# ut-amrl/nautilus

Measured on AMD Instinct MI355X. Metric: loop-closure candidate pairs/sec (1081-beam), higher is better.
Workload: dtype u16

## Files before the change

### nautilus_amd/csm.py

```python
import ctypes as C
import math

import numpy as np

from . import _lib
from ._lib import GridSpec, GridLayout, Search, Match, check, ptr

MATCH_DTYPE = np.dtype([("itheta", "<i4"), ("ix", "<i4"), ("iy", "<i4"), ("score", "<f4")])
assert MATCH_DTYPE.itemsize == C.sizeof(Match) == 16


def grid_spec(range_m=30.0, res=0.05, sigma=2.0, floor_p=1e-10, max_shift=40, cell_bits=16, skip_map=False, no_image=False):
    return GridSpec(float(range_m), float(res), float(sigma), float(floor_p), int(max_shift), int(cell_bits),
                    (_lib.NHIP_GRID_SKIP_MAP if skip_map else 0) | (_lib.NHIP_GRID_NO_IMAGE if no_image else 0), 0)


def search_spec(n_theta=61, nx=81, ny=81, theta_step=math.radians(1.0), exhaustive=False, dense=False, short_scans=False,
                exact_score=False, latency=False):
    flags = (_lib.NHIP_SEARCH_EXHAUSTIVE if exhaustive else 0) | (_lib.NHIP_SEARCH_DENSE if dense else 0) | \
            (_lib.NHIP_SEARCH_SHORT_SCANS if short_scans else 0) | (_lib.NHIP_SEARCH_EXACT_SCORE if exact_score else 0) | \
            (_lib.NHIP_SEARCH_LATENCY if latency else 0)
    return Search(int(n_theta), int(nx), int(ny), flags, float(theta_step))


# ... 174 lines not shown
    return np.asarray(matches)["itheta"] < 0


def gate_floor(spec, min_score, n_points):
    out = C.c_int32(0)
    check(_lib.load().nhip_csm_gate_floor(C.byref(spec), float(min_score), int(n_points), C.byref(out)))
    return out.value


def bnb_stats():
    a, b = C.c_uint64(0), C.c_uint64(0)
    check(_lib.load().nhip_bnb_stats(C.byref(a), C.byref(b)))
    return a.value, b.value


def bnb_stats_levels():
    v = (C.c_uint64 * 24)()
    check(_lib.load().nhip_bnb_stats_levels(v))
    return {"blocks_whole": v[0], "blocks_total": v[1], "candidates_refined": v[2], "sub_blocks": v[3],
            "clk_wave_phase3": v[4], "clk_origins": v[5], "clk_sub_bounds": v[6], "clk_exact": v[7],
            "clk_slowest_wave": v[8], "clk_seeds": v[9], "clk_bounds": v[10], "clk_wave_phase3_100MHz": v[11],
            "pairs_handed_over": v[12], "clk_wave_second_kernel": v[13], "pose_evals16": v[14],
            "pairs_settled_by_gate": v[15], "passes_l2_runs": v[16], "passes_per_cell_field": v[17],
            "passes_per_cell_capacity": v[18]}


def score_volume(scans, grids, src, slot, theta0, search, origin=(0, 0)):
    out = np.zeros((search.n_theta, search.nx, search.ny), dtype=np.int32)
    check(_lib.load().nhip_csm_scores(scans._h, grids._h, int(src), int(slot), float(theta0),
                                      int(origin[0]), int(origin[1]), C.byref(search), ptr(out)))
    return out


def match_to_transform(m, spec, search, theta0, origin=(0, 0)):
    tx = (origin[0] + int(m["ix"]) - (search.nx - 1) // 2) * spec.res
    ty = (origin[1] + int(m["iy"]) - (search.ny - 1) // 2) * spec.res
    th = theta0 + (int(m["itheta"]) - (search.n_theta - 1) // 2) * search.theta_step
    return np.float32(tx), np.float32(ty), np.float32(th)


class CorrelativeScanMatcher:

    def __init__(self, scanner_range, trans_range, low_res, high_res, sigma=2.0, cell_bits=16):
        self.params = _lib.CsmParams(float(scanner_range), float(trans_range), float(low_res), float(high_res),
                                     float(sigma), 1e-10, int(cell_bits), 0)

    def GetTransformation(self, pointcloud_a, pointcloud_b, rotation_a, rotation_b, rotation_restriction):
        a = np.ascontiguousarray(pointcloud_a, dtype=np.float32).reshape(-1, 2)
        b = np.ascontiguousarray(pointcloud_b, dtype=np.float32).reshape(-1, 2)
        score, tx, ty, th = C.c_double(0), C.c_float(0), C.c_float(0), C.c_float(0)
        check(_lib.load().nhip_csm_get_transformation(C.byref(self.params), ptr(a), len(a), ptr(b), len(b),
                                                      float(rotation_a), float(rotation_b), float(rotation_restriction),
                                                      C.byref(score), C.byref(tx), C.byref(ty), C.byref(th)))
        return score.value, ((np.float32(tx.value), np.float32(ty.value)), np.float32(th.value))


def last_launch():
    out = (C.c_int32 * 8)()
    check(_lib.load().nhip_csm_last_launch(out))
    form = {0: "fused", 1: "split, one round", 2: "split, rounds on one stream", 3: "split, rounds overlapped on the helper stream"}
    return {"form": form.get(out[0], "?"), "form_id": out[0], "pairs_per_round": out[1], "rounds_of_state": out[2],
            "rounds": out[3], "short_scans": bool(out[4]), "hand_over_kernel": bool(out[5]), "instrumented": bool(out[6] & 1),
            "l2_runs": bool(out[6] & 2), "n_pairs": out[7]}


def drop_in_cache_stats():
    v = [C.c_int64(0) for _ in range(4)]
    check(_lib.load().nhip_csm_cache_stats(*[C.byref(x) for x in v]))
    return dict(zip(("entries", "bytes", "hits", "misses"), (x.value for x in v)))


def drop_in_cache_clear():
    check(_lib.load().nhip_csm_cache_clear())


def drop_in_cache_configure(max_bytes):
    check(_lib.load().nhip_csm_cache_configure(int(max_bytes)))
```

### nautilus_amd/csrc/nhip_bnb.hip

```cpp
#include <atomic>
#include <mutex>
#include <type_traits>
#include <vector>

#ifndef NHIP_BNB_INSTR
#define NHIP_BNB_INSTR 0
#endif
#if NHIP_BNB_INSTR
#define csm_bnb_kernel csm_bnb_kernel_instr
#define csm_bnb_rot_kernel csm_bnb_rot_kernel_instr
#define launchers_product launchers_instr
#define BNB_STATS(P) ((P).stats)
#define BNB_TIMELINE(P) ((P).timeline)
#else
#define BNB_STATS(P) (static_cast<unsigned long long *>(nullptr))
#define BNB_TIMELINE(P) (static_cast<unsigned long long *>(nullptr))
#endif

#include "nhip_bnb_params.h"
#include "nhip_bnb_wave.h"
#include "nhip_bnb_origin.h"
#include "nhip_bnb_bounds.h"
#include "nhip_bnb_exact.h"

// ... 71 lines not shown
    return;
  }
#pragma unroll 1
  for (int q = 0; q < 4; q++) {
    const uint32_t b = q == 0 ? sb0 : (q == 1 ? sb1 : (q == 2 ? sb2 : sb3));
    if (b == 0u || b < best_sum_cached<GLOBAL>(best, bcopy)) continue;
    int dy, dx;
    const uint32_t total = sub_sums8(rsrc, pitch8, (uint32_t)P.hi_copy_bytes, org, nch, Y, X, q >> 1, q & 1, lane, &dy, &dx);
    const int32_t ix = BNB_B * X + BNB_B4 * (q & 1) + dx, iy = BNB_B * Y + BNB_B4 * (q >> 1) + dy;
    if (CB == 1) {
      const unsigned long long key = best_key(P, k, ix, iy, total, 8);
      wave_atomic_max(best, key, lane);
      if (GLOBAL) bcopy = max(bcopy, (uint32_t)(key >> 32));
    } else {
      n[3] += refine16<GLOBAL>(P, rsrc16, org, nch, n_pts, k, ix, iy, total, lane < 16, lane, best, bcopy);
    }
    n[2]++;
  }
}

struct PhaseClocks {
  long long org, strip, eval;
  uint32_t run_passes, cell_passes_field, cell_passes_full;
};

__device__ __forceinline__ void flush_stats(unsigned long long *stats, const uint32_t *n, int32_t pair, const PhaseClocks *clk) {
  if (n) {
    if (n[0]) atomicAdd(&stats[0], (unsigned long long)n[0]);
    if (n[1]) atomicAdd(&stats[2], (unsigned long long)n[1]);
    if (n[2]) atomicAdd(&stats[3], (unsigned long long)n[2]);
    if (n[3]) atomicAdd(&stats[14], (unsigned long long)n[3]);
    if (pair < BNB_STATS_PAIRS) atomicAdd(&stats[BNB_STATS_HEAD + pair], 4ull * n[0] + n[2]);
  }
  if (clk) {
    atomicAdd(&stats[5], (unsigned long long)clk->org);
    atomicAdd(&stats[6], (unsigned long long)clk->strip);
    atomicAdd(&stats[7], (unsigned long long)clk->eval);
    if (clk->run_passes) atomicAdd(&stats[16], (unsigned long long)clk->run_passes);
    if (clk->cell_passes_field) atomicAdd(&stats[17], (unsigned long long)clk->cell_passes_field);
    if (clk->cell_passes_full) atomicAdd(&stats[18], (unsigned long long)clk->cell_passes_full);
  }
}

template <int CB, bool GLOBAL, bool RUNS = false>
__device__ __forceinline__ void rotation_pass(const BnbParams &P, const PairCtx &C, int32_t k, uint32_t u0, uint32_t u1,
                                              unsigned long long m0, unsigned long long m1, int lane,
                                              unsigned long long *best, uint32_t *done, uint32_t *org,
                                              uint32_t (&n_work)[4], PhaseClocks &clk, uint32_t *runs = nullptr) {
  long long t_mark = 0;
  float cf, sf;
  rotation_k(P, C.pair, k, &cf, &sf);
  if (BNB_STATS(P)) t_mark = clock64();
  int32_t nrc = RUNS_NONE;
  const int32_t nch = cache_origins<RUNS>(P, C.pts, C.n_pts, cf, sf, C.cx, C.cy, lane, org, true, runs, RUNS && P.l2_runs != 0, &nrc);
  if (BNB_STATS(P)) clk.org += clock64() - t_mark;
  if (RUNS && BNB_STATS(P)) {
    clk.run_passes += nrc > 0 ? 1u : 0u;
    clk.cell_passes_field += nrc == RUNS_FIELD ? 1u : 0u;
    clk.cell_passes_full += nrc == RUNS_FULL ? 1u : 0u;
  }
  const __amdgpu_buffer_rsrc_t rsrc16 = CB == 1 ? uniform_rsrc(C.grid, P.grid_bytes + P.skip_bytes)
                                                : uniform_rsrc(C.grid + P.hi_offset + 2 * P.hi_copy_bytes, P.t16_bytes);
  const __amdgpu_buffer_rsrc_t rsrc = uniform_rsrc(C.grid + P.hi_offset, 2 * P.hi_copy_bytes);
  const uint32_t pitch8 = (uint32_t)P.hi_tpr;
  const __amdgpu_buffer_rsrc_t p4 = uniform_rsrc(C.grid + P.grid_bytes + P.skip_bytes + P.pool_bytes, P.pool4_bytes);
  while ((m0 | m1) != 0ull) {
    const int b0 = m0 ? (int)__builtin_ctzll(m0) : 64 + (int)__builtin_ctzll(m1);
    const int Y = b0 / NB, X0 = b0 - NB * Y;
    int len = 1;
    while (len < 3 && X0 + len < NB) {
      const int b = b0 + len;
      if (!(((b < 64 ? m0 >> b : m1 >> (b - 64)) & 1ull))) break;
      len++;
    }
    uint32_t sb[12];
    uint32_t bcopy = GLOBAL ? best_sum<true>(best) : 0u;
    if (P.levels >= 2) {
      if (BNB_STATS(P)) t_mark = clock64();
// ... 151 lines not shown
    }
    if ((uint32_t)(wbest >> 32) < (uint32_t)gfloor) wbest = 0ull;
  }
  uint32_t n_work[4] = {0u, 0u, 0u, 0u};
  PairCtx C;
  C.grid = grid;
  C.pts = pts;
  C.n_pts = n_pts;
  C.cx = cx;
  C.cy = cy;
  C.pair = pair;
  if (BY_ROT) {
    __syncthreads();
    uint32_t *org = s_org + wave * ORG_WAVE + lane;
    PhaseClocks clk = {0, 0, 0, 0u, 0u, 0u};
    long long t_busy = 0, t_wall = 0;
    const long long t_phase1 = BNB_STATS(P) ? clock64() : 0;
    if (BNB_TIMELINE(P) && threadIdx.x == 0 && pair < BNB_STATS_PAIRS) BNB_TIMELINE(P)[4 * pair + 1] = wall_clock64();
    const uint32_t xcd = bid & 7u;
    bool handed_over = false;
    enum { SEED, OWN };
    int state = SEED;
    bool heavy = false;
    for (;;) {
      bool have = false;
      int32_t k = 0;
      uint32_t u0 = 0u, u1 = 0u;
      unsigned long long m0 = 0ull, m1 = 0ull;
      uint32_t *done = nullptr;
      if (state == SEED) {
        if ((uint32_t)(wbest >> 32) != 0u) {
          const int32_t v = (int32_t)(wbest & 0xffu);
          const uint32_t ub = (uint32_t)(wbest >> 32);
          k = (int32_t)((uint32_t)wbest >> 8);
          u0 = v == lane ? ub : 0u;
          u1 = v == lane + 64 ? ub : 0u;
          m0 = v < 64 ? 1ull << v : 0ull;
          m1 = v < 64 ? 0ull : 1ull << (v - 64);
          done = s_U + k * 128;
          have = true;
        }
      } else if (state == OWN) {
        const int32_t rank = (int32_t)wave_fetch_add(s_qhead, 1u, lane);
        if (rank >= P.n_theta) break;
        k = (int32_t)s_order[rank];
        u0 = s_U[k * 128 + lane];
        u1 = s_U[k * 128 + 64 + lane];
        const uint32_t bsum = best_sum<false>(s_best);
        m0 = __ballot(u0 != 0u && u0 >= bsum);
        m1 = __ballot(u1 != 0u && u1 >= bsum && lane + 64 < NB * NB);
        if ((m0 | m1) == 0ull) continue;
        if (heavy && (uint32_t)rank >= P.keep_ranks) {
          const uint32_t lx = (xcd + (uint32_t)rank) & 7u;
          const uint32_t e = wave_fetch_add(P.rot_count + 8 * lx, 1u, lane);
          if (e < P.rot_cap) {
            if (lane < 4) {
              const unsigned long long M41 = (1ull << 41) - 1ull;
              const unsigned long long word = lane == 0   ? ((unsigned long long)(uint32_t)pair << 24) | (uint32_t)k
                                              : lane == 1 ? (m0 & M41)
                                              : lane == 2 ? ((m0 >> 41) | (m1 << 23)) & M41
                                                          : (m1 >> 18);
              P.rot_list[(size_t)lx * P.rot_cap + e].w[lane] = word;
            }
            handed_over = true;
            continue;
          }
        }
        have = true;
      }
      if (have) rotation_pass<CB, false>(P, C, k, u0, u1, m0, m1, lane, s_best, done, org, n_work, clk);
      if (state == SEED) {
        __syncthreads();
        if (BNB_TIMELINE(P) && threadIdx.x == 0 && pair < BNB_STATS_PAIRS) BNB_TIMELINE(P)[4 * pair + 2] = wall_clock64();
        if (BNB_STATS(P)) {
          t_busy = clock64();
          t_wall = wall_clock64();
        }
        for (int32_t kk = threadIdx.x; kk < P.n_theta; kk += THREADS) {
          const unsigned long long mine = s_kmax[kk];
          int32_t rank = 0;
          for (int32_t j = 0; j < P.n_theta; j++) rank += s_kmax[j] > mine ? 1 : 0;
          s_order[rank] = (uint32_t)kk;
        }
        if (P.rot_list || SPLIT) {
          const uint32_t bsum = best_sum<false>(s_best);
          uint32_t mine = 0u;
          for (int32_t kk = wave; kk < P.n_theta; kk += WAVES) {
            const uint32_t c0 = s_U[kk * 128 + lane], c1 = s_U[kk * 128 + 64 + lane];
            mine += (uint32_t)__builtin_popcountll(__ballot(c0 != 0u && c0 >= bsum)) +
                    (uint32_t)__builtin_popcountll(__ballot(c1 != 0u && c1 >= bsum && lane + 64 < NB * NB));
          }
          if (wave_leader(lane)) atomicAdd(s_qn, mine);
        }
        __syncthreads();
        if (SPLIT) {
          const uint32_t bsum = best_sum<false>(s_best);
          uint32_t *rows = P.ps_rows + (size_t)pair * (size_t)P.n_theta * 128u;
          uint32_t live = 0u;
          for (int32_t r = wave; r < P.n_theta; r += WAVES) {
            const uint32_t kk = s_order[r];
            const uint32_t kmax = (uint32_t)(s_kmax[kk] >> 32);
            if (kmax == 0u || kmax < bsum) break;
            live = (uint32_t)r + 1u;
            const uint32_t w1 = lane == 62 ? kmax : (lane == 63 ? kk : s_U[kk * 128 + 64 + lane]);
            rows[(size_t)r * 128u + lane] = s_U[kk * 128 + lane];
            rows[(size_t)r * 128u + 64 + lane] = w1;
          }
          if (live && wave_leader(lane)) atomicMax(s_qhead, live);
          __syncthreads();
          if (threadIdx.x == 0) {
            P.ps_count[pair] = *s_qn;
            P.ps_live[pair] = *s_qhead;
            P.ps_next[pair] = 0u;
          }
          break;
        }
        heavy = P.rot_list && *s_qn >= P.heavy_min;
        state = OWN;
      }
    }
    if (BNB_STATS(P) && lane == 0) {
      const long long now = clock64();
      atomicAdd(&BNB_STATS(P)[4], (unsigned long long)(now - t_busy));
      atomicAdd(&BNB_STATS(P)[11], (unsigned long long)(wall_clock64() - t_wall));
      flush_stats(BNB_STATS(P), nullptr, pair, &clk);
      atomicMax(s_slow, (unsigned long long)(now - t_busy));
      if (wave == 0) {
        atomicAdd(&BNB_STATS(P)[9], (unsigned long long)(t_busy - t_phase1));
        atomicAdd(&BNB_STATS(P)[10], (unsigned long long)(t_phase1 - t_start));
        if (handed_over) atomicAdd(&BNB_STATS(P)[12], 1ull);
      }
    }
  } else {
  if ((uint32_t)(wbest >> 32) != 0u) {
      const int32_t k = (int32_t)((uint32_t)wbest >> 8), v = (int32_t)(wbest & 0xffu);
      const int Y = v / NB, X = v - NB * Y;
// ... 169 lines not shown
constexpr int ORDER_THREADS = 256;
__global__ __launch_bounds__(ORDER_THREADS) void csm_bnb_order_spread_kernel(BnbParams P) {
  const int32_t p = (int32_t)(blockIdx.x * ORDER_THREADS + threadIdx.x);
  if (p >= P.n_pairs) return;
  const int32_t extra_slots = P.ps_work_stride - P.pairs_per_xcd;
  const int32_t home = p / P.pairs_per_xcd;
  P.ps_work[(size_t)home * P.ps_work_stride + extra_slots + (p - home * P.pairs_per_xcd)] = p;
  const uint32_t want = cand_shares(P, P.ps_count[p]) - 1u;
  uint32_t got = 0u;
  if (want) {
    const uint32_t t0 = atomicAdd(P.ps_ticket, want);
    for (uint32_t j = 0; j < want; j++) {
      const uint32_t e = t0 + j;
      if ((int32_t)(e >> 3) >= extra_slots) break;
      P.ps_work[(size_t)((e + (uint32_t)home + 1u) & 7u) * P.ps_work_stride + (e >> 3)] = p;
      got++;
    }
  }
  P.ps_nw[p] = 1u + got;
}

constexpr int CAND_WAVES = 4;
constexpr int CAND_THREADS = 64 * CAND_WAVES;
template <int CB>
__global__ __launch_bounds__(CAND_THREADS, CB == 2 ? 5 : 4) void csm_bnb_cand_kernel(BnbParams P) {
  __shared__ uint32_t s_org2[CAND_WAVES * ORG_WAVE];
  __shared__ uint32_t s_run2[CAND_WAVES * RUN_WAVE];
  __shared__ unsigned long long s_best2;
  __shared__ uint32_t s_next2;
  const int lane = threadIdx.x & 63;
  const uint32_t xcd = blockIdx.x & 7u, slot = blockIdx.x >> 3;
  if ((int32_t)slot >= P.ps_work_stride) return;
  const int32_t pair = P.ps_work[(size_t)xcd * P.ps_work_stride + slot];
  if (pair < 0) return;
  const uint32_t live = P.ps_live[pair];
  if (live == 0u) return;
  const bool shared = P.ps_nw[pair] > 1u;
  if (BNB_TIMELINE(P) && threadIdx.x == 0 && pair < BNB_STATS_PAIRS)
    atomicMin(&BNB_TIMELINE(P)[4 * (size_t)BNB_STATS_PAIRS + 2 + pair], wall_clock64());
  if (threadIdx.x == 0) {
    s_best2 = P.keys[pair];
    s_next2 = 0u;
  }
  __syncthreads();
  unsigned long long *best = shared ? &P.keys[pair] : &s_best2;
  uint32_t *next = shared ? &P.ps_next[pair] : &s_next2;
  const uint32_t *rows = P.ps_rows + (size_t)pair * (size_t)P.n_theta * 128u;
  uint32_t *org = s_org2 + (threadIdx.x >> 6) * ORG_WAVE + lane;
  uint32_t *runs = s_run2 + (threadIdx.x >> 6) * RUN_WAVE;
  PairCtx C;
  pair_context(P, pair, &C);
  uint32_t n_work[4] = {0u, 0u, 0u, 0u};
  PhaseClocks clk = {0, 0, 0, 0u, 0u, 0u};
  const long long t0 = BNB_STATS(P) ? clock64() : 0;
  for (;;) {
    const uint32_t rank = wave_fetch_add(next, 1u, lane);
    if (rank >= live) break;
    const uint32_t u0 = rows[(size_t)rank * 128u + lane], u1 = rows[(size_t)rank * 128u + 64 + lane];
    const uint32_t kmax = (uint32_t)__builtin_amdgcn_readlane((int)u1, 62);
    const int32_t k = __builtin_amdgcn_readlane((int)u1, 63);
    const uint32_t bsum = best_sum<true>(best);
    if (kmax < bsum) break;
    const unsigned long long m0 = __ballot(u0 != 0u && u0 >= bsum);
    const unsigned long long m1 = __ballot(u1 != 0u && u1 >= bsum && lane + 64 < NB * NB);
    if ((m0 | m1) == 0ull) continue;
    rotation_pass<CB, true, true>(P, C, k, u0, u1, m0, m1, lane, best, nullptr, org, n_work, clk, runs);
  }
  if (BNB_STATS(P) && lane == 0) {
    atomicAdd(&BNB_STATS(P)[13], (unsigned long long)(clock64() - t0));
    flush_stats(BNB_STATS(P), n_work, pair, &clk);
  }
  if (BNB_TIMELINE(P) && lane == 0 && pair < BNB_STATS_PAIRS)
    atomicMax(&BNB_TIMELINE(P)[5 * (size_t)BNB_STATS_PAIRS + 2 + pair], wall_clock64());
  if (!shared) {
    __syncthreads();
    if (threadIdx.x == 0) P.keys[pair] = s_best2;
  }
}

}

namespace bnb {

namespace {
template <int CB, bool PL, bool BR, bool SP = false>
int launch_main(const BnbParams &P, const BnbPlan &plan, hipStream_t s) {
  constexpr int THREADS = SP ? 64 * SPLIT_WAVES : BNB_THREADS;
  const size_t lds = lds_bytes((size_t)plan.lds_first, P.n_theta, SP);
  const int64_t blocks = (int64_t)P.pairs_per_xcd * 8;
  constexpr int MAX_DEV = 64;
  static std::atomic<size_t> lds_set[MAX_DEV];
  int dev = 0;
  if (hipGetDevice(&dev) != hipSuccess || dev < 0 || dev >= MAX_DEV) dev = -1;
  if (dev < 0 || lds > lds_set[dev].load(std::memory_order_relaxed)) {
    NHIP_TRY_HIP(hipFuncSetAttribute(reinterpret_cast<const void *>(csm_bnb_kernel<CB, PL, BR, SP>),
                                     hipFuncAttributeMaxDynamicSharedMemorySize, (int)lds));
    if (dev >= 0) lds_set[dev].store(lds, std::memory_order_relaxed);
  }
  hipLaunchKernelGGL((csm_bnb_kernel<CB, PL, BR, SP>), dim3((uint32_t)blocks), dim3(THREADS), lds, s, P);
  return NHIP_OK;
}
// ... 62 lines not shown
```

### nautilus_amd/csrc/nhip_bnb_host.hip

```cpp
#include <atomic>
#include <memory>
#include <mutex>
#include <vector>

#include "nhip_bnb_params.h"

namespace nhip {

using namespace bnb;

namespace {

size_t bnb_lds_first(const GridLayout &L, bool pool_lds) {
  const size_t pool = pool_lds ? (size_t)L.pool_bytes : 0;
  return pool > (size_t)ORG_LDS ? pool : (size_t)ORG_LDS;
}
size_t bnb_lds_bytes(const GridLayout &L, const nhip_search_t *search, bool pool_lds) {
  return lds_bytes(bnb_lds_first(L, pool_lds), search->n_theta, false);
}
constexpr size_t LDS_MAX = 160 * 1024;

struct TimerScope {
  int id;
  hipStream_t s;
// ... 28 lines not shown
  return BNB_WS_HEADER + 8 * (((n + 7) / 8) * 16 + 64) * (int64_t)sizeof(RotEntry);
}
int64_t bnb_workspace_bytes(int32_t n_pairs) {
  const int64_t n = n_pairs > 0 ? n_pairs : 0;
  nhip_search_t any = {};
  const int64_t m = n <= SPLIT_PAIRS ? n : 2 * SPLIT_PAIRS;
  const int64_t split = bnb_plan(GridLayout(), &any, (int32_t)n, 0).sized_split
                            ? BNB_WS_HEADER + split_state_bytes(m, m / 512 + 4, 64) : 0;
  return std::max(bnb_workspace_bytes_lists(n_pairs), split);
}

BnbPlan bnb_plan(const GridLayout &L, const nhip_search_t *search, int32_t n_pairs, int64_t workspace_bytes) {
  const auto is = [](const char *v, char c) { return v && v[0] == c; };
  const auto num = [](const char *name, int unset) { const char *v = tunable(name); return v ? atoi(v) : unset; };
  const char *force = tunable("NHIP_BNB_KERNELS");
  const char *sp = tunable("NHIP_BNB_SPLIT");
  const char *sbat = tunable("NHIP_BNB_SPLIT_BATCH");
  const char *smax = tunable("NHIP_BNB_SPLIT_MAX");
  BnbPlan p = {};
  p.n_pairs = n_pairs;
  p.cb = L.cb;
  p.levels = is(tunable("NHIP_BNB_LEVELS"), '1') ? 1 : 2;
  p.l2_runs = !is(tunable("NHIP_BNB_L2_RUNS"), '0');
  p.general_all = is(tunable("NHIP_BNB_QUEUE"), '1');
  static_assert(NHIP_SHORT_SCAN_POINTS == 64 * OCL, "the header's promise is the by-rotation form's limit");
  p.short_scans = (search->flags & NHIP_SEARCH_SHORT_SCANS) != 0 && !p.general_all && (uint32_t)(L.S + 2 * L.pad) < ORG_LIMIT;
  p.instrumented = is(tunable("NHIP_BNB_INSTRUMENT"), '1');
  p.stats = p.instrumented && is(tunable("NHIP_BNB_STATS"), '1');
  p.timeline = p.instrumented && is(tunable("NHIP_BNB_TIMELINE"), '1');
  p.sized_split = n_pairs >= SPLIT_MIN_PAIRS || (n_pairs > 0 && (is(sp, '1') || sbat));
  if (workspace_bytes > 0 && n_pairs > 0 && !p.general_all && !is(sp, '0') && !is(force, '2') &&
      (n_pairs >= SPLIT_MIN_PAIRS || is(sp, '1'))) {
    p.batch = sbat && atoi(sbat) > 0 ? atoi(sbat) : SPLIT_PAIRS;
    if (p.batch > n_pairs) p.batch = n_pairs;
    for (;;) {
      p.slot_bytes = (split_state_bytes(p.batch, 1, search->n_theta) + 511) & ~(int64_t)511;
      p.slots = (workspace_bytes - BNB_WS_HEADER - 512) / p.slot_bytes;
      const int64_t rounds = (n_pairs + p.batch - 1) / p.batch;
      if (p.slots >= (rounds < 2 ? rounds : 2) || p.batch <= 512) break;
      p.batch = p.batch / 2 > 512 ? p.batch / 2 : 512;
    }
    if (p.slots > SPLIT_RING) p.slots = SPLIT_RING;
    if (p.slots < 1) p.batch = 0;
    if (!sbat && p.batch > 0 && n_pairs > p.batch && (p.slots < 2 || p.batch < SPLIT_PAIRS)) p.batch = 0;
  }
  p.rounds = p.batch > 0 ? (n_pairs + p.batch - 1) / p.batch : 1;
// ... 37 lines not shown
  n->device = dev;
  hipError_t e = hipStreamCreateWithFlags(&n->stream, hipStreamNonBlocking);
  for (int i = 0; i < SPLIT_RING && e == hipSuccess; i++) {
    e = hipEventCreateWithFlags(&n->ea[i], hipEventDisableTiming);
    if (e == hipSuccess) e = hipEventCreateWithFlags(&n->eb[i], hipEventDisableTiming);
  }
  if (e != hipSuccess) {
    delete n;
    return hip_fail(e, "split form: helper stream / events", __FILE__, __LINE__);
  }
  *out = n;
  return NHIP_OK;
}
static void split_set_release(SplitSet *set) {
  if (!set) return;
  std::lock_guard<std::mutex> lock(g_split_mu);
  g_split_free.push_back(set);
}

static thread_local BnbPlan t_last_plan = {};
void bnb_last_launch(int32_t out[8]) {
  const BnbPlan &p = t_last_plan;
  const int32_t info[8] = {p.form, (int32_t)p.batch, (int32_t)p.slots, (int32_t)p.rounds, p.short_scans, p.second,
                           (int32_t)p.instrumented | ((int32_t)p.l2_runs << 1), p.n_pairs};
  memcpy(out, info, sizeof(info));
}

static void fill_bnb_params(BnbParams &P, const MatchJob &job, const BnbPlan &plan) {
  const GridLayout &L = *job.L;
  fill_job_params(P, job);
  P.pair_kbase = job.pair_kbase;
  P.keys = reinterpret_cast<unsigned long long *>(job.keys);
  P.gate = job_gate(job);
  P.nbx = (P.nx + BNB_B - 1) / BNB_B;
  P.nby = (P.ny + BNB_B - 1) / BNB_B;
  P.pool_pitch = L.pool_pitch;
  P.pool_rows = L.pool_rows;
  P.pairs_per_xcd = (plan.n_pairs + 7) / 8;
  P.skip_bytes = L.skip_bytes;
  P.pool_bytes = L.pool_bytes;
  P.pool4_bytes = L.pool4_bytes;
  P.pool4_pitch = L.pool4_pitch;
  P.hi_offset = L.hi_offset;
  P.hi_bytes = L.hi_bytes;
  P.hi_pitch = L.hi_pitch;
  P.hi_tpr = L.hi_tpr;
  P.hi_copy_bytes = L.hi_copy_bytes;
  P.t16_bytes = L.t16_bytes;
  P.t16_tpr = L.t16_tpr;
  P.inv_res_f = (float)P.inv_res;
  P.levels = plan.levels;
  P.l2_runs = plan.l2_runs;
  P.general_all = plan.general_all;
  P.short_scans = plan.short_scans;
  P.heavy_min = plan.heavy_min;
  P.keep_ranks = plan.keep_ranks;
  P.rot_cap = plan.rot_cap;
  P.lds_first = (int32_t)plan.lds_first;
}

static int instr_buffers(const BnbPlan &plan, BnbParams &P, hipStream_t s) {
  if (!plan.stats && !plan.timeline) return NHIP_OK;
  std::lock_guard<std::mutex> lock(g_instr_mu);
  if (plan.stats) {
    if (!g_bnb_stats) {
      NHIP_TRY_HIP(hipMalloc(reinterpret_cast<void **>(&g_bnb_stats), 8 * (BNB_STATS_HEAD + (size_t)BNB_STATS_PAIRS)));
      NHIP_TRY_HIP(hipMemset(g_bnb_stats, 0, 8 * (BNB_STATS_HEAD + (size_t)BNB_STATS_PAIRS)));
    }
    P.stats = g_bnb_stats;
  }
  if (plan.timeline) {
    if (!g_bnb_timeline) NHIP_TRY_HIP(hipMalloc(reinterpret_cast<void **>(&g_bnb_timeline), 48 * (size_t)BNB_STATS_PAIRS + 16));
    P.timeline = g_bnb_timeline;
    NHIP_TRY_HIP(hipMemsetAsync(g_bnb_timeline + 4 * (size_t)BNB_STATS_PAIRS + 2, 0xff, 8 * (size_t)BNB_STATS_PAIRS, s));
    NHIP_TRY_HIP(hipMemsetAsync(g_bnb_timeline + 5 * (size_t)BNB_STATS_PAIRS + 2, 0, 8 * (size_t)BNB_STATS_PAIRS, s));
// ... 135 lines not shown
```

### nautilus_amd/csrc/nhip_bnb_origin.h

```cpp
#pragma once
#include "nhip_bnb_params.h"
#include "nhip_bnb_wave.h"

namespace nhip {
namespace {

using namespace bnb;

template <bool LEAN = false>
__device__ __forceinline__ void window_origin(float2 q, float cf, float sf, const BnbParams &P, int32_t cx, int32_t cy,
                                              int32_t *prow, int32_t *pcol) {
  const float xr = __fsub_rn(__fmul_rn(cf, q.x), __fmul_rn(sf, q.y));
  const float yr = __fadd_rn(__fmul_rn(sf, q.x), __fmul_rn(cf, q.y));
  const int32_t half = P.S / 2;
  const bool finite __attribute__((unused)) = (fabsf(xr) < 1e9f) && (fabsf(yr) < 1e9f);
  int32_t ix, iy;
  const float mx = __fmul_rn(xr, P.inv_res_f), my = __fmul_rn(yr, P.inv_res_f);
  const float fx = floorf(mx), fy = floorf(my);
  if (LEAN) {
    const float rx = __fsub_rn(mx, fx), ry = __fsub_rn(my, fy);
    const float dx = fminf(rx, __fsub_rn(1.0f, rx)), dy = fminf(ry, __fsub_rn(1.0f, ry));
    const float tx = __fmul_rn(fabsf(mx), 0x1p-22f), ty = __fmul_rn(fabsf(my), 0x1p-22f);
    const unsigned long long slow = __builtin_amdgcn_fcmpf(dx, tx, 13 ) | __builtin_amdgcn_fcmpf(dy, ty, 13 );
    ix = (int32_t)fx;
// ... 68 lines not shown
  if (live) {
    int32_t prow, pcol;
    window_origin(q, cf, sf, P, cx, cy, &prow, &pcol);
    const int32_t col = pcol + BNB_B * X;
    *g = (uint32_t)((prow + BNB_B * Y) * P.pitch + (col & ~3));
    *sh = (uint32_t)(col & 3) * 8u;
  }
}


constexpr int ORG_COL_SHIFT = 6, ORG_ROW_SHIFT = 19;
__device__ __forceinline__ uint32_t org_row(uint32_t o) { return o >> ORG_ROW_SHIFT; }
__device__ __forceinline__ uint32_t org_col(uint32_t o) { return (o >> ORG_COL_SHIFT) & (ORG_LIMIT - 1u); }
__device__ __forceinline__ uint32_t org_cnt(uint32_t o) { return (o & 63u) + 1u; }

__device__ __forceinline__ uint32_t origin_of(const uint32_t *org, int c) { return c < OCL ? org[64 * c] : 0u; }

constexpr uint32_t RUN_KEY_MASK = (~0u << (ORG_ROW_SHIFT + 2)) | (((ORG_LIMIT >> 2) - 1u) << (ORG_COL_SHIFT + 2));
__device__ __forceinline__ uint32_t run_row2(uint32_t e) { return e >> (ORG_ROW_SHIFT + 2); }
__device__ __forceinline__ uint32_t run_col2(uint32_t e) { return (e >> (ORG_COL_SHIFT + 2)) & ((ORG_LIMIT >> 2) - 1u); }
__device__ __forceinline__ uint32_t run_cnt(uint32_t e) { return e & 127u; }
enum : int32_t { RUNS_NONE = 0, RUNS_FIELD = -1, RUNS_FULL = -2 };

template <bool RUNS = false>
__device__ __forceinline__ int32_t cache_origins(const BnbParams &P, const float2 *pts, int32_t n_pts, float cf, float sf,
                                                 int32_t cx, int32_t cy, int lane, uint32_t *org, bool merged,
                                                 uint32_t *runs = nullptr, bool want_runs = false,
                                                 int32_t *run_chunks = nullptr) {
  uint32_t *base = org - lane;
  const bool with_runs = RUNS && want_runs;
  if (RUNS) *run_chunks = RUNS_NONE;
  for (int merge = merged ? 1 : 0; merge >= 0; merge--) {
    constexpr int D = 6;
    float px[D], py[D];
#pragma unroll
    for (int d = 0; d < D; d++) {
      const float2 q = 64 * d + lane < n_pts ? pts[64 * d + lane] : make_float2(0.f, 0.f);
      px[d] = q.x;
      py[d] = q.y;
    }
    uint32_t tail = 0u;
    uint32_t rtail = 0u;
#pragma unroll 1
    for (int c = 0; c < OCL; c++) {
      const int32_t idx = 64 * c + lane;
      if (64 * c >= n_pts) break;
      const float2 pt = make_float2(px[0], py[0]);
      const float2 qn = idx + 64 * D < n_pts ? pts[idx + 64 * D] : make_float2(0.f, 0.f);
#pragma unroll
      for (int d = 0; d < D - 1; d++) {
        px[d] = px[d + 1];
// ... 9 lines not shown
        o = ((uint32_t)prow << ORG_ROW_SHIFT) | ((uint32_t)pcol << ORG_COL_SHIFT);
      }
      const uint32_t prev = (uint32_t)__builtin_amdgcn_update_dpp((int)o, (int)o, 0x138 , 0xF, 0xF, false);
      const bool head = live && (lane == 0 || o != prev || merge == 0);
      const unsigned long long H = __ballot(head), L = __ballot(live);
      const unsigned long long rest = ((H | ~L) >> lane) >> 1;
      const uint32_t cnt = rest ? (uint32_t)__builtin_ctzll(rest) + 1u : (uint32_t)(64 - lane);
      if (head) {
        const uint32_t before = __builtin_amdgcn_mbcnt_hi((uint32_t)(H >> 32), __builtin_amdgcn_mbcnt_lo((uint32_t)H, 0u));
        base[tail + before] = o | (cnt - 1u);
      }
      tail += (uint32_t)__builtin_popcountll(H);
      if (RUNS && with_runs && merge) {
        const bool head2 = live && (lane == 0 || ((o ^ prev) & RUN_KEY_MASK) != 0u);
        const unsigned long long H2 = __ballot(head2);
        const unsigned long long rest2 = ((H2 | ~L) >> lane) >> 1;
        const uint32_t cnt2 = rest2 ? (uint32_t)__builtin_ctzll(rest2) + 1u : (uint32_t)(64 - lane);
        const uint32_t at = rtail + __builtin_amdgcn_mbcnt_hi((uint32_t)(H2 >> 32), __builtin_amdgcn_mbcnt_lo((uint32_t)H2, 0u));
        if (head2 && at < (uint32_t)RUN_WAVE) runs[at] = (o & RUN_KEY_MASK) | cnt2;
        rtail += (uint32_t)__builtin_popcountll(H2);
      }
    }
    const int32_t nch = (int32_t)((tail + 63u) >> 6);
    for (uint32_t e = tail + (uint32_t)lane; e < (uint32_t)ORG_WAVE; e += 64u) base[e] = 0u;
    if (RUNS && with_runs && merge)
      for (uint32_t e = rtail + (uint32_t)lane; e < (uint32_t)RUN_WAVE; e += 64u) runs[e] = 0u;
    __builtin_amdgcn_fence(__ATOMIC_RELEASE, "wavefront");
    __builtin_amdgcn_wave_barrier();
    if (merge == 0) {
      if (RUNS && with_runs) *run_chunks = RUNS_FIELD;
      return nch;
    }
    uint32_t w = 0u;
    for (int c = 0; c < nch; c++) {
      const uint32_t e = org[64 * c];
      w += 64u * (uint32_t)c + (uint32_t)lane < tail ? org_cnt(e) : 0u;
    }
    w = sum8(w);
    if (__ballot(w > 257u) == 0ull) {
      if (RUNS && with_runs) {
        const int32_t nrc = (int32_t)((rtail + 63u) >> 6);
        uint32_t w2 = 0u;
        if (rtail <= (uint32_t)RUN_WAVE)
          for (int c = 0; c < nrc; c++) w2 += run_cnt(runs[64 * c + lane]);
        w2 = sum8(w2);
        *run_chunks = rtail > (uint32_t)RUN_WAVE ? RUNS_FULL : (__ballot(w2 > 257u) != 0ull ? RUNS_FIELD : nrc);
      }
      return nch;
    }
    __builtin_amdgcn_wave_barrier();
  }
  return 0;
}

}
}
```

### nautilus_amd/csrc/nhip_bnb_params.h

```cpp
#pragma once
#include "nhip_common.h"
#include "nhip_csm_shared.h"

namespace nhip {
namespace bnb {

constexpr int BNB_WAVES = 8;
constexpr int NB = BNB_MAX_NB;
constexpr int MAX_ROT = 340;
constexpr int QCAP = 1024;
constexpr int SPLIT_WAVES = 8;
constexpr int LIST_ENTRIES = 128;
constexpr int RUN_SHIFT = 25;
constexpr int OC = 18;
constexpr int OCL = 17;
constexpr int ORG_WAVE = OCL * 64;
constexpr int ORG_LDS = BNB_WAVES * ORG_WAVE * 4;
constexpr uint32_t ORG_LIMIT = 1u << 13;
constexpr int RUN_CHUNKS = 8;
constexpr int RUN_WAVE = RUN_CHUNKS * 64;

constexpr int QSPACE_SPLIT = (SPLIT_WAVES * LIST_ENTRIES * 4 + MAX_ROT * 12 + 15) / 16 * 2;
constexpr int lds_qspace(bool split) { return split ? QSPACE_SPLIT : QCAP; }
static_assert(QSPACE_SPLIT <= QCAP, "the split form's LDS must not exceed the fused form's, which bnb_fits() checks");
// ... 46 lines not shown
  uint32_t split_min;
  uint32_t split_max;
  uint32_t front_min;
  int32_t pair_base;
  int32_t n_pairs, n_theta, nx, ny, hx, hy, nbx, nby;
  int32_t S, pad, pitch, rows, max_shift;
  int32_t pool_pitch, pool_rows, pairs_per_xcd;
  int32_t pool4_pitch;
  int32_t lds_first;
  int32_t general_all;
  int32_t short_scans;
  int32_t levels;
  int64_t grid_bytes, skip_bytes, slot_bytes, pool_bytes, pool4_bytes;
  int64_t hi_offset, hi_bytes;
  int32_t hi_pitch;
  int32_t hi_tpr;
  int64_t hi_copy_bytes;
  int64_t t16_bytes;
  int32_t t16_tpr;
  double res, inv_res;
  float inv_res_f;
  ScoreGate gate;
  int32_t l2_runs;
};

using BnbLaunch = int (*)(const BnbParams &P, const BnbPlan &plan, hipStream_t s);
struct BnbLaunchers { BnbLaunch fused, split_a, split_b; };
BnbLaunchers launchers_product();
BnbLaunchers launchers_instr();

}
}
```

### nautilus_amd/csrc/nhip_common.h

```cpp
#pragma once
#include <hip/hip_runtime.h>

#include <cmath>
#include <cstdint>
#include <cstdio>
#include <cstring>
#include <string>
#include <vector>

#include "../../include/nautilus_hip_debug.h"

namespace nhip {

void set_error(const char *fmt, ...);
int hip_fail(hipError_t e, const char *what, const char *file, int line);

#define NHIP_TRY_HIP(expr)                                            \
  do {                                                                \
    hipError_t _e = (expr);                                           \
    if (_e != hipSuccess) return ::nhip::hip_fail(_e, #expr, __FILE__, __LINE__); \
  } while (0)

#define NHIP_REQUIRE(cond, ...)          \
  do {                                   \
// ... 123 lines not shown
int launch_grid_build(const float *d_xy, const int32_t *d_offsets, int32_t n_scans, const int32_t *d_target_ids,
                      int32_t n_targets, const nhip_grid_spec_t *spec, const GridLayout &L,
                      uint8_t *d_grids, void *d_ws, int64_t ws_bytes, hipStream_t s, bool incremental = false);

enum MatchForm : int32_t {
  MATCH_BNB,
  MATCH_POSES,
  MATCH_STRIPS8,
  MATCH_STRIPS16,
};
struct MatchPlan {
  MatchForm form = MATCH_BNB;
  int32_t tile_rows = 0, n_tiles = 0;
  bool keys_zeroed = false, keys_undecoded = false;
};
MatchPlan csm_plan(const GridLayout &L, const nhip_search_t *search, int32_t n_pairs);

enum BnbForm : int32_t { BNB_FUSED, BNB_SPLIT_ONE, BNB_SPLIT_ROUNDS, BNB_SPLIT_OVERLAP };
struct BnbPlan {
  BnbForm form;
  int32_t n_pairs, cb, levels;
  bool second, general_all, short_scans, pool_lds, instrumented, stats, timeline;
  bool l2_runs;
  bool sized_split;
  uint32_t rot_cap, heavy_min, keep_ranks, split_min, split_max;
  int64_t batch, slots, slot_bytes, rounds;
  int64_t lds_first;
};
BnbPlan bnb_plan(const GridLayout &L, const nhip_search_t *search, int32_t n_pairs, int64_t workspace_bytes);

struct MatchJob {
  const float *xy = nullptr;
  const int32_t *offsets = nullptr;
  IdBounds ids = {0, 0, nullptr};
  const uint8_t *grids = nullptr;
  const nhip_grid_spec_t *spec = nullptr;
  const GridLayout *L = nullptr;
  const int32_t *pair_src = nullptr, *pair_slot = nullptr;
  const double *rot0_cs = nullptr;
  const double *delta_cs = nullptr;
  const int32_t *pair_origin = nullptr, *pair_kbase = nullptr;
  int32_t n_pairs = 0;
  const nhip_search_t *search = nullptr;
  double min_score = -INFINITY;
  uint64_t *keys = nullptr;
  nhip_match_t *out = nullptr;
// ... 147 lines not shown
```

Before: 1.637 million.

## Hand seed-pass origin lists to the candidate kernel instead of recomputing them

In the split form, the first kernel's seed rotation pass now records its computed origin list and stores it into spare rows of the per-pair buffer, along with a packed descriptor word, when space allows. The second (candidate) kernel loads that stored list for the matching rotation instead of re-rotating and re-binning all scan points, then rebuilds the run-length list from it. This removes redundant origin caching work at the cost of extra global stores/loads, packing logic, and a ballot/readlane fit check. An instrumented build cross-checks stored lists against recomputed ones.

```diff
diff --git a/nautilus_amd/csm.py b/nautilus_amd/csm.py
--- a/nautilus_amd/csm.py
+++ b/nautilus_amd/csm.py
@@ -220,7 +220,8 @@
             "clk_slowest_wave": v[8], "clk_seeds": v[9], "clk_bounds": v[10], "clk_wave_phase3_100MHz": v[11],
             "pairs_handed_over": v[12], "clk_wave_second_kernel": v[13], "pose_evals16": v[14],
             "pairs_settled_by_gate": v[15], "passes_l2_runs": v[16], "passes_per_cell_field": v[17],
-            "passes_per_cell_capacity": v[18]}
+            "passes_per_cell_capacity": v[18], "passes_stored_origins": v[19], "seed_lists_written": v[20],
+            "stored_origin_mismatches": v[21]}
 
 
 def score_volume(scans, grids, src, slot, theta0, search, origin=(0, 0)):
@@ -259,7 +260,7 @@
     form = {0: "fused", 1: "split, one round", 2: "split, rounds on one stream", 3: "split, rounds overlapped on the helper stream"}
     return {"form": form.get(out[0], "?"), "form_id": out[0], "pairs_per_round": out[1], "rounds_of_state": out[2],
             "rounds": out[3], "short_scans": bool(out[4]), "hand_over_kernel": bool(out[5]), "instrumented": bool(out[6] & 1),
-            "l2_runs": bool(out[6] & 2), "n_pairs": out[7]}
+            "l2_runs": bool(out[6] & 2), "seed_origins": bool(out[6] & 4), "n_pairs": out[7]}
 
 
 def drop_in_cache_stats():
diff --git a/nautilus_amd/csrc/nhip_bnb.hip b/nautilus_amd/csrc/nhip_bnb.hip
--- a/nautilus_amd/csrc/nhip_bnb.hip
+++ b/nautilus_amd/csrc/nhip_bnb.hip
@@ -117,6 +117,7 @@
 struct PhaseClocks {
   long long org, strip, eval;
   uint32_t run_passes, cell_passes_field, cell_passes_full;
+  uint32_t stored_passes, stored_mismatch;
 };
 
 __device__ __forceinline__ void flush_stats(unsigned long long *stats, const uint32_t *n, int32_t pair, const PhaseClocks *clk) {
@@ -134,21 +135,43 @@
     if (clk->run_passes) atomicAdd(&stats[16], (unsigned long long)clk->run_passes);
     if (clk->cell_passes_field) atomicAdd(&stats[17], (unsigned long long)clk->cell_passes_field);
     if (clk->cell_passes_full) atomicAdd(&stats[18], (unsigned long long)clk->cell_passes_full);
-  }
-}
-
-template <int CB, bool GLOBAL, bool RUNS = false>
+    if (clk->stored_passes) atomicAdd(&stats[19], (unsigned long long)clk->stored_passes);
+    if (clk->stored_mismatch) atomicAdd(&stats[21], (unsigned long long)clk->stored_mismatch);
+  }
+}
+
+enum { SEEDS_OFF, SEEDS_TELL, SEEDS_TAKE };
+template <int CB, bool GLOBAL, bool RUNS = false, int SEEDS = SEEDS_OFF>
 __device__ __forceinline__ void rotation_pass(const BnbParams &P, const PairCtx &C, int32_t k, uint32_t u0, uint32_t u1,
                                               unsigned long long m0, unsigned long long m1, int lane,
                                               unsigned long long *best, uint32_t *done, uint32_t *org,
-                                              uint32_t (&n_work)[4], PhaseClocks &clk, uint32_t *runs = nullptr) {
+                                              uint32_t (&n_work)[4], PhaseClocks &clk, uint32_t *runs = nullptr,
+                                              uint32_t *seed = nullptr, const uint32_t *region = nullptr,
+                                              uint32_t *chk = nullptr) {
   long long t_mark = 0;
   float cf, sf;
   rotation_k(P, C.pair, k, &cf, &sf);
   if (BNB_STATS(P)) t_mark = clock64();
   int32_t nrc = RUNS_NONE;
-  const int32_t nch = cache_origins<RUNS>(P, C.pts, C.n_pts, cf, sf, C.cx, C.cy, lane, org, true, runs, RUNS && P.l2_runs != 0, &nrc);
+  int32_t nch;
+  const bool stored = SEEDS == SEEDS_TAKE && *seed != SEED_NONE;
+  if (SEEDS == SEEDS_TAKE && stored)
+    nch = load_origins<RUNS>(region, *seed, lane, org, runs, RUNS && P.l2_runs != 0, &nrc);
+  else
+    nch = cache_origins<RUNS, SEEDS == SEEDS_TELL>(P, C.pts, C.n_pts, cf, sf, C.cx, C.cy, lane, org, true, runs,
+                                                   RUNS && P.l2_runs != 0, &nrc, seed);
   if (BNB_STATS(P)) clk.org += clock64() - t_mark;
+  if (NHIP_BNB_INSTR && SEEDS == SEEDS_TAKE && RUNS && BNB_STATS(P) && stored) {
+    int32_t nrc2 = RUNS_NONE;
+    const int32_t nch2 = cache_origins<RUNS>(P, C.pts, C.n_pts, cf, sf, C.cx, C.cy, lane, chk + lane, true, chk + ORG_WAVE,
+                                             P.l2_runs != 0, &nrc2);
+    uint32_t bad = 0u;
+    for (int e = lane; e < ORG_WAVE; e += 64) bad += (org - lane)[e] != chk[e] ? 1u : 0u;
+    if (nrc > 0 || nrc2 > 0)
+      for (int e = lane; e < RUN_WAVE; e += 64) bad += runs[e] != chk[ORG_WAVE + e] ? 1u : 0u;
+    clk.stored_mismatch += wave_sum(bad) + (nch2 != nch ? 1u : 0u) + (nrc2 != nrc ? 1u : 0u);
+    clk.stored_passes++;
+  }
   if (RUNS && BNB_STATS(P)) {
     clk.run_passes += nrc > 0 ? 1u : 0u;
     clk.cell_passes_field += nrc == RUNS_FIELD ? 1u : 0u;
@@ -346,6 +369,7 @@
     enum { SEED, OWN };
     int state = SEED;
     bool heavy = false;
+    uint32_t seed_told = SEED_NONE;
     for (;;) {
       bool have = false;
       int32_t k = 0;
@@ -392,7 +416,9 @@
         }
         have = true;
       }
-      if (have) rotation_pass<CB, false>(P, C, k, u0, u1, m0, m1, lane, s_best, done, org, n_work, clk);
+      if (SPLIT) {
+        if (have) rotation_pass<CB, false, false, SEEDS_TELL>(P, C, k, u0, u1, m0, m1, lane, s_best, done, org, n_work, clk, nullptr, &seed_told);
+      } else if (have) rotation_pass<CB, false>(P, C, k, u0, u1, m0, m1, lane, s_best, done, org, n_work, clk);
       if (state == SEED) {
         __syncthreads();
         if (BNB_TIMELINE(P) && threadIdx.x == 0 && pair < BNB_STATS_PAIRS) BNB_TIMELINE(P)[4 * pair + 2] = wall_clock64();
@@ -405,6 +431,7 @@
           int32_t rank = 0;
           for (int32_t j = 0; j < P.n_theta; j++) rank += s_kmax[j] > mine ? 1 : 0;
           s_order[rank] = (uint32_t)kk;
+          if (SPLIT) s_list[WAVES + kk] = (uint32_t)rank;
         }
         if (P.rot_list || SPLIT) {
           const uint32_t bsum = best_sum<false>(s_best);
@@ -431,11 +458,45 @@
             rows[(size_t)r * 128u + 64 + lane] = w1;
           }
           if (live && wave_leader(lane)) atomicMax(s_qhead, live);
+          if (P.seed_origins) {
+            uint32_t mine = SEED_NONE;
+            if (seed_told != SEED_NONE) mine = (s_list[WAVES + ((uint32_t)wbest >> 8)] << 8) | (((seed_told >> 1) + 63u) >> 6);
+            if (wave_leader(lane)) s_list[wave] = mine;
+          }
           __syncthreads();
+          uint32_t stored_mask = 0u;
+          if (P.seed_origins) {
+            const uint32_t live_all = *s_qhead;
+            const uint32_t mine = lane < WAVES ? s_list[lane] : SEED_NONE;
+            const bool eligible = mine != SEED_NONE && (mine >> 8) < live_all;
+            uint32_t upto = 0u;
+#pragma unroll
+            for (int j = 0; j < WAVES; j++) {
+              const uint32_t other = (uint32_t)__builtin_amdgcn_readlane((int)mine, j);
+              if (other != SEED_NONE && (other >> 8) < live_all && (other >> 8) <= (mine >> 8)) upto += other & 255u;
+            }
+            const bool fits = eligible && 2u * live_all + upto <= 2u * (uint32_t)P.n_theta - 1u;
+            stored_mask = (uint32_t)__ballot(fits) & ((1u << WAVES) - 1u);
+            const int w = __builtin_amdgcn_readfirstlane(wave);
+            if ((stored_mask >> w) & 1u) {
+              const uint32_t nch = (((seed_told >> 1) + 63u) >> 6);
+              const uint32_t chunk0 = 2u * live_all + (uint32_t)__builtin_amdgcn_readlane((int)upto, w) - nch;
+              const __amdgpu_buffer_rsrc_t lrs = uniform_rsrc(rows + (size_t)chunk0 * 64u, 256 * (int64_t)nch);
+              uint32_t v[OCL];
+#pragma unroll
+              for (int c = 0; c < OCL; c++) v[c] = org[64 * c];
+#pragma unroll
+              for (int c = 0; c < OCL; c++)
+                if (c < (int)nch) __builtin_amdgcn_raw_buffer_store_b32(v[c], lrs, 4 * (64 * c + lane), 0, SEED_STORE_AUX);
+              if (wave_leader(lane))
+                rows[(size_t)P.n_theta * 128u - WAVES + w] = seed_word((uint32_t)wbest >> 8, seed_told >> 1, (seed_told & 1u) != 0u, chunk0);
+            }
+          }
           if (threadIdx.x == 0) {
             P.ps_count[pair] = *s_qn;
-            P.ps_live[pair] = *s_qhead;
+            P.ps_live[pair] = *s_qhead | (stored_mask << 16);
             P.ps_next[pair] = 0u;
+            if (stats_g && stored_mask) atomicAdd(&stats_g[20], (unsigned long long)__builtin_popcount(stored_mask));
           }
           break;
         }
@@ -651,6 +712,10 @@
 
 constexpr int CAND_WAVES = 4;
 constexpr int CAND_THREADS = 64 * CAND_WAVES;
+#if NHIP_BNB_INSTR
+#pragma clang diagnostic push
+#pragma clang diagnostic ignored "-Wpass-failed"
+#endif
 template <int CB>
 __global__ __launch_bounds__(CAND_THREADS, CB == 2 ? 5 : 4) void csm_bnb_cand_kernel(BnbParams P) {
   __shared__ uint32_t s_org2[CAND_WAVES * ORG_WAVE];
@@ -662,7 +727,8 @@
   if ((int32_t)slot >= P.ps_work_stride) return;
   const int32_t pair = P.ps_work[(size_t)xcd * P.ps_work_stride + slot];
   if (pair < 0) return;
-  const uint32_t live = P.ps_live[pair];
+  const uint32_t live_word = P.ps_live[pair];
+  const uint32_t live = live_word & 0xffffu;
   if (live == 0u) return;
   const bool shared = P.ps_nw[pair] > 1u;
   if (BNB_TIMELINE(P) && threadIdx.x == 0 && pair < BNB_STATS_PAIRS)
@@ -677,6 +743,14 @@
   const uint32_t *rows = P.ps_rows + (size_t)pair * (size_t)P.n_theta * 128u;
   uint32_t *org = s_org2 + (threadIdx.x >> 6) * ORG_WAVE + lane;
   uint32_t *runs = s_run2 + (threadIdx.x >> 6) * RUN_WAVE;
+  uint32_t seed_dir = SEED_NONE;
+  if (lane < SPLIT_WAVES && ((live_word >> (16 + lane)) & 1u)) seed_dir = rows[(size_t)P.n_theta * 128u - SPLIT_WAVES + lane];
+#if NHIP_BNB_INSTR
+  __shared__ uint32_t s_chk2[CAND_WAVES * (ORG_WAVE + RUN_WAVE)];
+  uint32_t *chk = s_chk2 + (threadIdx.x >> 6) * (ORG_WAVE + RUN_WAVE);
+#else
+  uint32_t *chk = nullptr;
+#endif
   PairCtx C;
   pair_context(P, pair, &C);
   uint32_t n_work[4] = {0u, 0u, 0u, 0u};
@@ -693,7 +767,9 @@
     const unsigned long long m0 = __ballot(u0 != 0u && u0 >= bsum);
     const unsigned long long m1 = __ballot(u1 != 0u && u1 >= bsum && lane + 64 < NB * NB);
     if ((m0 | m1) == 0ull) continue;
-    rotation_pass<CB, true, true>(P, C, k, u0, u1, m0, m1, lane, best, nullptr, org, n_work, clk, runs);
+    uint32_t seed = (uint32_t)__builtin_amdgcn_readlane((int)seed_dir, k & (SPLIT_WAVES - 1));
+    if (seed_k(seed) != (uint32_t)k) seed = SEED_NONE;
+    rotation_pass<CB, true, true, SEEDS_TAKE>(P, C, k, u0, u1, m0, m1, lane, best, nullptr, org, n_work, clk, runs, &seed, rows, chk);
   }
   if (BNB_STATS(P) && lane == 0) {
     atomicAdd(&BNB_STATS(P)[13], (unsigned long long)(clock64() - t0));
@@ -706,6 +782,9 @@
     if (threadIdx.x == 0) P.keys[pair] = s_best2;
   }
 }
+#if NHIP_BNB_INSTR
+#pragma clang diagnostic pop
+#endif
 
 }
 
diff --git a/nautilus_amd/csrc/nhip_bnb_host.hip b/nautilus_amd/csrc/nhip_bnb_host.hip
--- a/nautilus_amd/csrc/nhip_bnb_host.hip
+++ b/nautilus_amd/csrc/nhip_bnb_host.hip
@@ -74,6 +74,7 @@
   p.cb = L.cb;
   p.levels = is(tunable("NHIP_BNB_LEVELS"), '1') ? 1 : 2;
   p.l2_runs = !is(tunable("NHIP_BNB_L2_RUNS"), '0');
+  p.seed_origins = !is(tunable("NHIP_BNB_SEED_ORIGINS"), '0');
   p.general_all = is(tunable("NHIP_BNB_QUEUE"), '1');
   static_assert(NHIP_SHORT_SCAN_POINTS == 64 * OCL, "the header's promise is the by-rotation form's limit");
   p.short_scans = (search->flags & NHIP_SEARCH_SHORT_SCANS) != 0 && !p.general_all && (uint32_t)(L.S + 2 * L.pad) < ORG_LIMIT;
@@ -157,7 +158,7 @@
 void bnb_last_launch(int32_t out[8]) {
   const BnbPlan &p = t_last_plan;
   const int32_t info[8] = {p.form, (int32_t)p.batch, (int32_t)p.slots, (int32_t)p.rounds, p.short_scans, p.second,
-                           (int32_t)p.instrumented | ((int32_t)p.l2_runs << 1), p.n_pairs};
+                           (int32_t)p.instrumented | ((int32_t)p.l2_runs << 1) | ((int32_t)p.seed_origins << 2), p.n_pairs};
   memcpy(out, info, sizeof(info));
 }
 
@@ -186,6 +187,7 @@
   P.inv_res_f = (float)P.inv_res;
   P.levels = plan.levels;
   P.l2_runs = plan.l2_runs;
+  P.seed_origins = plan.seed_origins;
   P.general_all = plan.general_all;
   P.short_scans = plan.short_scans;
   P.heavy_min = plan.heavy_min;
diff --git a/nautilus_amd/csrc/nhip_bnb_origin.h b/nautilus_amd/csrc/nhip_bnb_origin.h
--- a/nautilus_amd/csrc/nhip_bnb_origin.h
+++ b/nautilus_amd/csrc/nhip_bnb_origin.h
@@ -114,11 +114,43 @@
 __device__ __forceinline__ uint32_t run_cnt(uint32_t e) { return e & 127u; }
 enum : int32_t { RUNS_NONE = 0, RUNS_FIELD = -1, RUNS_FULL = -2 };
 
-template <bool RUNS = false>
+__device__ __forceinline__ void org_zero_tail(uint32_t *base, uint32_t tail, int lane) {
+  for (uint32_t e = tail + (uint32_t)lane; e < (uint32_t)ORG_WAVE; e += 64u) base[e] = 0u;
+}
+__device__ __forceinline__ void runs_zero_tail(uint32_t *runs, uint32_t rtail, int lane) {
+  for (uint32_t e = rtail + (uint32_t)lane; e < (uint32_t)RUN_WAVE; e += 64u) runs[e] = 0u;
+}
+__device__ __forceinline__ void lists_written() {
+  __builtin_amdgcn_fence(__ATOMIC_RELEASE, "wavefront");
+  __builtin_amdgcn_wave_barrier();
+}
+__device__ __forceinline__ int32_t runs_outcome(const uint32_t *runs, uint32_t rtail, int lane) {
+  const int32_t nrc = (int32_t)((rtail + 63u) >> 6);
+  uint32_t w2 = 0u;
+  if (rtail <= (uint32_t)RUN_WAVE)
+    for (int c = 0; c < nrc; c++) w2 += run_cnt(runs[64 * c + lane]);
+  w2 = sum8(w2);
+  return rtail > (uint32_t)RUN_WAVE ? RUNS_FULL : (__ballot(w2 > 257u) != 0ull ? RUNS_FIELD : nrc);
+}
+
+constexpr uint32_t SEED_NONE = 0xffffffffu;
+constexpr int SEED_STORE_AUX = 16 | 2, SEED_LOAD_AUX = 2;
+__device__ __forceinline__ uint32_t seed_word(uint32_t k, uint32_t tail, bool merged, uint32_t chunk0) {
+  const uint32_t nch = (tail + 63u) >> 6;
+  return k | (nch << 9) | ((merged ? 1u : 0u) << 14) | (chunk0 << 15) | (((tail - 1u) & 63u) << 25);
+}
+__device__ __forceinline__ uint32_t seed_k(uint32_t w) { return w & 511u; }
+__device__ __forceinline__ uint32_t seed_nch(uint32_t w) { return (w >> 9) & 31u; }
+__device__ __forceinline__ bool seed_merged(uint32_t w) { return ((w >> 14) & 1u) != 0u; }
+__device__ __forceinline__ uint32_t seed_chunk0(uint32_t w) { return (w >> 15) & 1023u; }
+__device__ __forceinline__ uint32_t seed_tail(uint32_t w) { return 64u * (seed_nch(w) - 1u) + ((w >> 25) & 63u) + 1u; }
+static_assert(MAX_ROT < 511 && 2 * MAX_ROT < 1024 && OCL < 32, "the fields of a seed's word hold every list");
+
+template <bool RUNS = false, bool TELL = false>
 __device__ __forceinline__ int32_t cache_origins(const BnbParams &P, const float2 *pts, int32_t n_pts, float cf, float sf,
                                                  int32_t cx, int32_t cy, int lane, uint32_t *org, bool merged,
                                                  uint32_t *runs = nullptr, bool want_runs = false,
-                                                 int32_t *run_chunks = nullptr) {
+                                                 int32_t *run_chunks = nullptr, uint32_t *told = nullptr) {
   uint32_t *base = org - lane;
   const bool with_runs = RUNS && want_runs;
   if (RUNS) *run_chunks = RUNS_NONE;
@@ -174,11 +206,10 @@
       }
     }
     const int32_t nch = (int32_t)((tail + 63u) >> 6);
-    for (uint32_t e = tail + (uint32_t)lane; e < (uint32_t)ORG_WAVE; e += 64u) base[e] = 0u;
-    if (RUNS && with_runs && merge)
-      for (uint32_t e = rtail + (uint32_t)lane; e < (uint32_t)RUN_WAVE; e += 64u) runs[e] = 0u;
-    __builtin_amdgcn_fence(__ATOMIC_RELEASE, "wavefront");
-    __builtin_amdgcn_wave_barrier();
+    org_zero_tail(base, tail, lane);
+    if (RUNS && with_runs && merge) runs_zero_tail(runs, rtail, lane);
+    lists_written();
+    if (TELL) *told = (tail << 1) | (uint32_t)merge;
     if (merge == 0) {
       if (RUNS && with_runs) *run_chunks = RUNS_FIELD;
       return nch;
@@ -190,14 +221,7 @@
     }
     w = sum8(w);
     if (__ballot(w > 257u) == 0ull) {
-      if (RUNS && with_runs) {
-        const int32_t nrc = (int32_t)((rtail + 63u) >> 6);
-        uint32_t w2 = 0u;
-        if (rtail <= (uint32_t)RUN_WAVE)
-          for (int c = 0; c < nrc; c++) w2 += run_cnt(runs[64 * c + lane]);
-        w2 = sum8(w2);
-        *run_chunks = rtail > (uint32_t)RUN_WAVE ? RUNS_FULL : (__ballot(w2 > 257u) != 0ull ? RUNS_FIELD : nrc);
-      }
+      if (RUNS && with_runs) *run_chunks = runs_outcome(runs, rtail, lane);
       return nch;
     }
     __builtin_amdgcn_wave_barrier();
@@ -205,5 +229,61 @@
   return 0;
 }
 
-}
-}
+__device__ __forceinline__ uint32_t wave_scan(uint32_t v) {
+  v += (uint32_t)__builtin_amdgcn_update_dpp(0, (int)v, 0x111, 0xF, 0xF, false);
+  v += (uint32_t)__builtin_amdgcn_update_dpp(0, (int)v, 0x112, 0xF, 0xF, false);
+  v += (uint32_t)__builtin_amdgcn_update_dpp(0, (int)v, 0x114, 0xF, 0xF, false);
+  v += (uint32_t)__builtin_amdgcn_update_dpp(0, (int)v, 0x118, 0xF, 0xF, false);
+  v += (uint32_t)__builtin_amdgcn_update_dpp(0, (int)v, 0x142, 0xA, 0xF, false);
+  return v + (uint32_t)__builtin_amdgcn_update_dpp(0, (int)v, 0x143, 0xC, 0xF, false);
+}
+
+template <bool RUNS = false>
+__device__ __forceinline__ int32_t load_origins(const uint32_t *region, uint32_t w, int lane, uint32_t *org,
+                                                uint32_t *runs = nullptr, bool want_runs = false,
+                                                int32_t *run_chunks = nullptr) {
+  const int32_t nch = (int32_t)seed_nch(w);
+  const uint32_t tail = seed_tail(w);
+  const bool with_runs = RUNS && want_runs;
+  const __amdgpu_buffer_rsrc_t rs = uniform_rsrc(region + 64u * seed_chunk0(w), 256 * (int64_t)nch);
+  uint32_t v[OCL];
+#pragma unroll
+  for (int c = 0; c < OCL; c++) v[c] = __builtin_amdgcn_raw_buffer_load_b32(rs, 4 * (64 * c + lane), 0, SEED_LOAD_AUX);
+#pragma unroll
+  for (int c = 0; c < OCL; c++) org[64 * c] = c < nch ? v[c] : 0u;
+  if (RUNS) *run_chunks = RUNS_NONE;
+  if (!(RUNS && with_runs && seed_merged(w))) {
+    lists_written();
+    if (RUNS && with_runs) *run_chunks = RUNS_FIELD;
+    return nch;
+  }
+  lists_written();
+  uint32_t rtail = 0u, points = 0u, last = 0u;
+  uint32_t ahead = org[0];
+#pragma unroll 1
+  for (int c = 0; c < nch; c++) {
+    const uint32_t e = ahead;
+    ahead = org[64 * (c + 1 < OCL ? c + 1 : OCL - 1)];
+    const bool live = 64u * (uint32_t)c + (uint32_t)lane < tail;
+    const uint32_t cnt = live ? org_cnt(e) : 0u;
+    const uint32_t upto = wave_scan(cnt);
+    uint32_t prev = (uint32_t)__builtin_amdgcn_update_dpp((int)e, (int)e, 0x138 , 0xF, 0xF, false);
+    prev = lane == 0 ? last : prev;
+    const bool head = live && ((((points + upto - cnt) & 63u) == 0u) | (((e ^ prev) & RUN_KEY_MASK) != 0u));
+    const unsigned long long H = __ballot(head);
+    const uint32_t heads = __builtin_amdgcn_mbcnt_hi((uint32_t)(H >> 32), __builtin_amdgcn_mbcnt_lo((uint32_t)H, 0u));
+    const uint32_t at = rtail + heads - (head ? 0u : 1u);
+    if (head && at < (uint32_t)RUN_WAVE) runs[at] = (e & RUN_KEY_MASK) | cnt;
+    if (live && !head && at < (uint32_t)RUN_WAVE) __hip_atomic_fetch_add(&runs[at], cnt, __ATOMIC_RELAXED, __HIP_MEMORY_SCOPE_WORKGROUP);
+    rtail += (uint32_t)__builtin_popcountll(H);
+    points += (uint32_t)__builtin_amdgcn_readlane((int)upto, 63);
+    last = (uint32_t)__builtin_amdgcn_readlane((int)e, 63);
+  }
+  runs_zero_tail(runs, rtail, lane);
+  lists_written();
+  *run_chunks = runs_outcome(runs, rtail, lane);
+  return nch;
+}
+
+}
+}
diff --git a/nautilus_amd/csrc/nhip_bnb_params.h b/nautilus_amd/csrc/nhip_bnb_params.h
--- a/nautilus_amd/csrc/nhip_bnb_params.h
+++ b/nautilus_amd/csrc/nhip_bnb_params.h
@@ -92,6 +92,7 @@
   float inv_res_f;
   ScoreGate gate;
   int32_t l2_runs;
+  int32_t seed_origins;
 };
 
 using BnbLaunch = int (*)(const BnbParams &P, const BnbPlan &plan, hipStream_t s);
diff --git a/nautilus_amd/csrc/nhip_common.h b/nautilus_amd/csrc/nhip_common.h
--- a/nautilus_amd/csrc/nhip_common.h
+++ b/nautilus_amd/csrc/nhip_common.h
@@ -169,6 +169,7 @@
   int32_t n_pairs, cb, levels;
   bool second, general_all, short_scans, pool_lds, instrumented, stats, timeline;
   bool l2_runs;
+  bool seed_origins;
   bool sized_split;
   uint32_t rot_cap, heavy_min, keep_ranks, split_min, split_max;
   int64_t batch, slots, slot_bytes, rounds;
```

Result: no change. 1.648 million, median of 6 (+0.7%).
